# kubernetes-sigs/scheduler-plugins

Hardware: AMD Instinct MI355X
Metric: pod_x_node_filter_score_evals_per_sec (higher is better)
Workload: dtype f32+f64

## Files before the change

scheduler-plugins_amd/csrc/kernels_network.hip:

```cpp
#include <cstdlib>

#include "net_device.h"

namespace spx {

namespace {

using Acc = AccT<int>;


constexpr int kRowThreads = kNetRowThreads;
__global__ __launch_bounds__(kRowThreads) void k_net_cls(NetArgs g) {
  SPX_RESOLVE_ROWS(g);
  extern __shared__ __align__(16) int lds[];
  const int C = g.n_classes;
  int* cls_word = lds;
  int* cls_hosts = lds + C;
  uint32_t* cls_fin = reinterpret_cast<uint32_t*>(lds + 2 * C);
  unsigned* host_bits = reinterpret_cast<unsigned*>(lds + 3 * C);
  const int lane = threadIdx.x, nthr = blockDim.x;
  const int64_t pod = g.row_begin + blockIdx.x;
  if (pod >= g.row_end) return;
  const int key = g.pod_key[pod];
  const int flag = g.key_flag[key];
  const int lo = g.pair_ptr[key], hi = g.pair_end ? g.pair_end[key] : g.pair_ptr[key + 1];
  const int64_t n_words = (g.n_nodes + 31) / 32;
  const uint8_t* other0 = g.other_status[0] ? g.other_status[0] + pod * g.row_stride : nullptr;
  const uint8_t* other1 = g.other_status[1] ? g.other_status[1] + pod * g.row_stride : nullptr;
  uint8_t* out_st = g.out_status + pod * g.row_stride;
  uint8_t* out_sc = g.out_score + pod * g.row_stride;

  constexpr int kG = 16;
  const int64_t groups = g.row_stride / kG;
  uint16_t* scored = reinterpret_cast<uint16_t*>(host_bits + n_words);
  const bool fuse = g.out_alloc != nullptr && nthr == 64;
  uint8_t* out_al = fuse ? g.out_alloc + pod * g.row_stride : nullptr;
  auto load16 = [](const void* p) { return *reinterpret_cast<const uint4*>(p); };
  auto byte_of = [](const uint32_t (&w)[4], int j) { return (w[j >> 2] >> (8 * (j & 3))) & 0xffu; };
  auto half_of = [](const uint32_t (&w)[8], int j) { return (w[j >> 1] >> (16 * (j & 1))) & 0xffffu; };
  auto rel16 = [&](int64_t n0, uint32_t (&r)[16]) {
#pragma unroll
    for (int q = 0; q < 4; ++q) {
      const uint4 v = load16(g.alloc_rel + n0 + 4 * q);
      r[4 * q] = v.x, r[4 * q + 1] = v.y, r[4 * q + 2] = v.z, r[4 * q + 3] = v.w;
    }
  };
  auto others16 = [&](int64_t n0, uint32_t (&oth)[4]) {
    uint4 o4 = uint4{0, 0, 0, 0};
    if (other0) o4 = load16(other0 + n0);
    if (other1) {
      const uint4 v = load16(other1 + n0);
      o4.x |= v.x, o4.y |= v.y, o4.z |= v.z, o4.w |= v.w;
    }
    oth[0] = o4.x, oth[1] = o4.y, oth[2] = o4.z, oth[3] = o4.w;
  };
  auto open16 = [&](int64_t n0, const uint32_t (&oth)[4]) {
    uint32_t open = 0;
#pragma unroll
    for (int j = 0; j < kG; ++j) open |= (n0 + j < g.n_nodes && byte_of(oth, j) == 0u) ? 1u << j : 0u;
    return open;
  };
  auto wave_range = [&](uint32_t& lo32, uint32_t& hi32) {
    lo32 = static_cast<uint32_t>(wave_min(static_cast<int>(lo32 ^ 0x80000000u))) ^ 0x80000000u;
    hi32 = static_cast<uint32_t>(wave_max(static_cast<int>(hi32 ^ 0x80000000u))) ^ 0x80000000u;
  };
  auto alloc16 = [&](int64_t n0, uint32_t ok, uint32_t alo, double ab, uint32_t (&al_w)[4]) {
    uint32_t rel[16];
    rel16(n0, rel);
#pragma unroll
    for (int j = 0; j < kG; ++j)
      if ((ok >> j) & 1u) al_w[j >> 2] |= static_cast<uint32_t>(static_cast<double>(rel[j] - alo) * ab) << (8 * (j & 3));
  };

  if (flag != 0) {
    const uint32_t st = flag == 2 ? 0xffffffffu : 0u;
    uint32_t alo = 0xffffffffu, ahi = 0u;
    const bool fz = fuse && flag != 2;
    if (fz) {
      for (int64_t q = lane; q < groups; q += nthr) {
        const int64_t n0 = q * kG;
        uint32_t open = 0;
        if (n0 < g.n_nodes) {
          uint32_t oth[4], rel[16];
          others16(n0, oth);
          rel16(n0, rel);
          open = open16(n0, oth);
#pragma unroll
          for (int j = 0; j < kG; ++j)
            if ((open >> j) & 1u) alo = rel[j] < alo ? rel[j] : alo, ahi = rel[j] > ahi ? rel[j] : ahi;
        }
        scored[q] = static_cast<uint16_t>(open);
      }
      wave_range(alo, ahi);
    }
    const uint32_t arange = (fz && ahi >= alo) ? ahi - alo : 0u;
    const double ab = arange ? (100.0 / static_cast<double>(arange)) * (1.0 + 0x1p-49) : 0.0;
    for (int64_t q = lane; q < groups; q += nthr) {
      const int64_t n0 = q * kG;
      *reinterpret_cast<uint4*>(out_st + n0) = uint4{st, st, st, st};
      *reinterpret_cast<uint4*>(out_sc + n0) = uint4{0u, 0u, 0u, 0u};
      if (fuse) {
        uint32_t al_w[4] = {0, 0, 0, 0};
        const uint32_t ok = fz ? scored[q] : 0u;
        if (ok != 0 && arange != 0) alloc16(n0, ok, alo, ab, al_w);
        *reinterpret_cast<uint4*>(out_al + n0) = uint4{al_w[0], al_w[1], al_w[2], al_w[3]};
      }
    }
    return;
  }

  constexpr int kStage = kNetStagePairs;
  const int scored_words = static_cast<int>((g.row_stride / 16 + 1) / 2);
  long long* sp_max = reinterpret_cast<long long*>(lds + ((3 * C + static_cast<int>(n_words) + scored_words + 1) & ~1));
  int* sp_host = reinterpret_cast<int*>(sp_max + kStage);
  int* sp_region = sp_host + kStage;
  int* sp_zone = sp_region + kStage;
  const bool staged = nthr == kRowThreads && hi - lo <= kStage;
  const StagedPairs sp{sp_host, sp_region, sp_zone, sp_max, hi - lo};
  if (staged) {
    for (int i = lane; i < hi - lo; i += nthr) {
      const int host = g.pair_node[lo + i];
      sp_host[i] = host, sp_region[i] = g.region[host], sp_zone[i] = g.zone[host], sp_max[i] = g.pair_max[lo + i];
    }
    __syncthreads();
  }
  auto direct = [&](int64_t node) { return staged ? direct_eval_staged<int>(g, node, sp) : direct_eval<int>(g, node, lo, hi); };
  for (int c = lane; c < C; c += nthr) {
    Acc a{0, 0, 0};
    const int region = g.cls_region[c], zone = g.cls_zone[c];
    if (staged) {
      for (int i = 0; i < sp.n; ++i) add_pair(a, g, region, zone, sp_region[i], sp_zone[i], sp_max[i]);
    } else {
      for (int i = lo; i < hi; ++i) {
        const int host = g.pair_node[i];
        add_pair(a, g, region, zone, g.region[host], g.zone[host], g.pair_max[i]);
      }
    }
    cls_word[c] = a.cost | (a.vio > a.sat ? static_cast<int>(0x80000000u) : 0);
    cls_hosts[c] = 0;
  }
  for (int64_t w = lane; w < n_words; w += nthr) host_bits[w] = 0u;
  __syncthreads();
  for (int i = lo + lane; i < hi; i += nthr) {
    const int host = g.pair_node[i];
    const unsigned bit = 1u << (host & 31);
    if (!(atomicOr(&host_bits[host >> 5], bit) & bit)) atomicAdd(&cls_hosts[g.node_class16[host]], 1);
  }
  __syncthreads();

  auto classes16 = [&](int64_t n0, uint32_t (&cw)[8]) {
    const uint4 c0 = load16(g.node_class16 + n0), c1 = load16(g.node_class16 + n0 + 8);
    cw[0] = c0.x, cw[1] = c0.y, cw[2] = c0.z, cw[3] = c0.w, cw[4] = c1.x, cw[5] = c1.y, cw[6] = c1.z, cw[7] = c1.w;
  };
  auto hosts16 = [&](int64_t n0) -> uint32_t { return (host_bits[n0 >> 5] >> (n0 & 31)) & 0xffffu; };

  int mn = INT32_MAX, mx = INT32_MIN;
  uint32_t alo = 0xffffffffu, ahi = 0u;
  const bool walk = other0 || other1 || fuse;
  if (!walk) {
    for (int c = lane; c < C; c += nthr) {
      const int w = cls_word[c];
      if (w >= 0 && g.cls_size[c] - cls_hosts[c] > 0) {
        mn = w < mn ? w : mn;
        mx = w > mx ? w : mx;
      }
    }
    for (int i = lo + lane; i < hi; i += nthr) {
      const Acc a = direct(g.pair_node[i]);
      if (!(a.vio > a.sat)) {
        mn = a.cost < mn ? a.cost : mn;
        mx = a.cost > mx ? a.cost : mx;
      }
    }
  } else {
    for (int64_t q = lane; q < groups; q += nthr) {
      const int64_t n0 = q * kG;
      uint32_t ok = 0;
      if (n0 < g.n_nodes) {
        uint32_t oth[4], cw[8], rel[16];
        others16(n0, oth);
        classes16(n0, cw);
        if (fuse) rel16(n0, rel);
        const uint32_t hb = hosts16(n0);
        const uint32_t open = open16(n0, oth);
#pragma unroll
        for (int j = 0; j < kG; ++j) {
          const int w = cls_word[half_of(cw, j)];
          if (((open & ~hb) >> j) & 1u && w >= 0) {
            mn = w < mn ? w : mn;
            mx = w > mx ? w : mx;
            ok |= 1u << j;
            if (fuse) alo = rel[j] < alo ? rel[j] : alo, ahi = rel[j] > ahi ? rel[j] : ahi;
          }
        }
        for (uint32_t hs = open & hb; hs != 0; hs &= hs - 1) {
          const int j = __builtin_ctz(hs);
          const Acc a = direct(n0 + j);
          if (!(a.vio > a.sat)) {
            mn = a.cost < mn ? a.cost : mn;
            mx = a.cost > mx ? a.cost : mx;
            ok |= 1u << j;
            if (fuse) {
              const uint32_t r = g.alloc_rel[n0 + j];
              alo = r < alo ? r : alo, ahi = r > ahi ? r : ahi;
            }
          }
        }
      }
      scored[q] = static_cast<uint16_t>(ok);
    }
  }
  mn = wave_min(mn);
  mx = wave_max(mx);
  if (fuse) wave_range(alo, ahi);
  if (nthr > 64) {
    __shared__ int s_mn[kRowThreads / 64], s_mx[kRowThreads / 64];
    if ((lane & 63) == 0) s_mn[lane >> 6] = mn, s_mx[lane >> 6] = mx;
    __syncthreads();
    mn = INT32_MAX, mx = INT32_MIN;
    for (int w = 0; w < (nthr >> 6); ++w) {
      mn = s_mn[w] < mn ? s_mn[w] : mn;
      mx = s_mx[w] > mx ? s_mx[w] : mx;
    }
  }

  for (int c = lane; c < C; c += nthr) {
    const int w = cls_word[c];
    int score = w >= 0 ? norm_cost(w, mn, mx) : 0;
    score = score < 0 ? 0 : (score > 255 ? 255 : score);
    cls_fin[c] = static_cast<uint32_t>(score) | (w < 0 ? static_cast<uint32_t>(SPX_NET_ST_UNSCHEDULABLE) << 8 : 0u);
  }
  __syncthreads();
  const uint32_t arange = (fuse && ahi >= alo) ? ahi - alo : 0u;
  const double ab = arange ? (100.0 / static_cast<double>(arange)) * (1.0 + 0x1p-49) : 0.0;

  for (int64_t q = lane; q < groups; q += nthr) {
    const int64_t n0 = q * kG;
    uint32_t st_w[4] = {0, 0, 0, 0}, sc_w[4] = {0, 0, 0, 0}, al_w[4] = {0, 0, 0, 0};
    if (n0 < g.n_nodes) {
      const uint32_t ok = walk ? scored[q] : 0xffffu;
      uint32_t cw[8];
      classes16(n0, cw);
      const uint32_t hb = hosts16(n0);
#pragma unroll
      for (int j = 0; j < kG; ++j) {
        uint32_t fin = cls_fin[half_of(cw, j)];
        if (n0 + j >= g.n_nodes) fin = 0;
        st_w[j >> 2] |= (fin >> 8) << (8 * (j & 3));
        if ((ok >> j) & 1u) sc_w[j >> 2] |= (fin & 0xffu) << (8 * (j & 3));
      }
      for (uint32_t hs = hb; hs != 0; hs &= hs - 1) {
        const int j = __builtin_ctz(hs);
        if (n0 + j >= g.n_nodes) continue;
        const Acc a = direct(n0 + j);
        const bool pass = !(a.vio > a.sat);
        int score = pass ? norm_cost(a.cost, mn, mx) : 0;
        score = score < 0 ? 0 : (score > 255 ? 255 : score);
        const uint32_t sh = 8 * (j & 3), keep = ~(0xffu << sh);
        st_w[j >> 2] = (st_w[j >> 2] & keep) | ((pass ? 0u : static_cast<uint32_t>(SPX_NET_ST_UNSCHEDULABLE)) << sh);
        sc_w[j >> 2] = (sc_w[j >> 2] & keep) | ((((ok >> j) & 1u) ? static_cast<uint32_t>(score) : 0u) << sh);
      }
      if (fuse && ok != 0 && arange != 0) alloc16(n0, ok, alo, ab, al_w);
    }
    *reinterpret_cast<uint4*>(out_st + n0) = uint4{st_w[0], st_w[1], st_w[2], st_w[3]};
    *reinterpret_cast<uint4*>(out_sc + n0) = uint4{sc_w[0], sc_w[1], sc_w[2], sc_w[3]};
    if (fuse) *reinterpret_cast<uint4*>(out_al + n0) = uint4{al_w[0], al_w[1], al_w[2], al_w[3]};
  }
}

}

size_t net_lds_bytes(int n_classes, int64_t n_nodes) {
  return static_cast<size_t>(3 * n_classes) * sizeof(int) + static_cast<size_t>((n_nodes + 31) / 32) * sizeof(unsigned) +
         static_cast<size_t>((n_nodes + 4096) / 16 + 2) * sizeof(uint16_t) + 16;
}

bool launch_net(const NetArgs& g, hipStream_t s) {
  if (g.row_end <= g.row_begin) return false;
  if (g.cost_wide) {
    launch_net_wide(g, s);
    return false;
  }
  const unsigned blocks = static_cast<unsigned>(g.row_end - g.row_begin);
  size_t lds = g.n_classes > 0 ? net_lds_bytes(g.n_classes, g.n_nodes) : 16;
  if (blocks == 1) lds = ((lds + 7) & ~static_cast<size_t>(7)) + kNetStagePairs * (sizeof(long long) + 3 * sizeof(int));
  const bool generic_only = (g.opts & kOptNetGeneric) != 0;
  if (!generic_only && !g.out_raw && g.n_classes > 0 && g.n_classes <= 65535 && g.node_class16 && g.row_stride % 16 == 0) {
    NetArgs h = g;
    if (blocks == 1 || !h.alloc_rel) h.out_alloc = nullptr;
    hipLaunchKernelGGL(k_net_cls, dim3(blocks), dim3(blocks == 1 ? kRowThreads : 64), lds, s, h);
    return h.out_alloc != nullptr;
  }
  hipLaunchKernelGGL(k_net<int>, dim3(blocks), dim3(64), lds, s, g);
  return false;
}

}
```

Measured before the change: 4923 billion.

## Add templated multi-row class kernel with software-pipelined 16-node group loads

Adds a new per-row network kernel, templated on which other-status inputs exist and whether allocation scoring is fused, and launches it for multi-row batches. It processes 16-node groups with vector loads and double-buffers status, class and alloc-rel loads one burst ahead, computing min/max with branchless masks. The aim is to hide global load latency and remove runtime branches and per-byte work from the old generic path. In exchange it adds eight kernel instantiations, more register pressure, and a separate host-node fixup loop that must reproduce the old semantics exactly.

```diff
diff --git a/scheduler-plugins_amd/csrc/kernels_network.hip b/scheduler-plugins_amd/csrc/kernels_network.hip
--- a/scheduler-plugins_amd/csrc/kernels_network.hip
+++ b/scheduler-plugins_amd/csrc/kernels_network.hip
@@ -268,6 +268,343 @@
   }
 }
 
+constexpr int kGrp = 16;
+constexpr int kBurst = 4;
+constexpr int kBurstW = 1;
+
+__device__ __forceinline__ uint4 ld16(const void* p) { return *reinterpret_cast<const uint4*>(p); }
+__device__ __forceinline__ uint32_t word_of(const uint4& v, int i) { return i == 0 ? v.x : (i == 1 ? v.y : (i == 2 ? v.z : v.w)); }
+__device__ __forceinline__ uint32_t half16(const uint4& c0, const uint4& c1, int j) {
+  return (word_of(j < 8 ? c0 : c1, (j & 7) >> 1) >> (16 * (j & 1))) & 0xffffu;
+}
+__device__ __forceinline__ uint32_t mask_of_bit(uint32_t bits, int j) { return static_cast<uint32_t>(static_cast<int>(bits << (31 - j)) >> 31); }
+__device__ __forceinline__ uint32_t umin32(uint32_t a, uint32_t b) { return a < b ? a : b; }
+__device__ __forceinline__ uint32_t umax32(uint32_t a, uint32_t b) { return a > b ? a : b; }
+__device__ __forceinline__ uint32_t nonzero_bytes(uint32_t x) {
+  x |= x >> 4, x |= x >> 2, x |= x >> 1;
+  return ((x & 0x01010101u) * 0x01020408u) >> 24 & 0xfu;
+}
+__device__ __forceinline__ void pin(uint32_t& x) { asm volatile("" : "+v"(x)); }
+__device__ __forceinline__ void put_byte(uint4& v, int j, uint32_t b) {
+  const uint32_t s = b << (8 * (j & 3));
+  if ((j >> 2) == 0) v.x |= s;
+  else if ((j >> 2) == 1) v.y |= s;
+  else if ((j >> 2) == 2) v.z |= s;
+  else v.w |= s;
+}
+
+template <bool kO0, bool kO1, bool kFuse>
+__global__ __launch_bounds__(64) void k_net_cls_rows(NetArgs g) {
+  SPX_RESOLVE_ROWS(g);
+  extern __shared__ __align__(16) int lds[];
+  const int C = g.n_classes;
+  int* cls_word = lds;
+  int* cls_hosts = lds + C;
+  uint32_t* cls_fin = reinterpret_cast<uint32_t*>(lds + 2 * C);
+  unsigned* host_bits = reinterpret_cast<unsigned*>(lds + 3 * C);
+  const int lane = threadIdx.x;
+  const int64_t pod = g.row_begin + blockIdx.x;
+  if (pod >= g.row_end) return;
+  const int key = g.pod_key[pod];
+  const int flag = g.key_flag[key];
+  const int lo = g.pair_ptr[key], hi = g.pair_end ? g.pair_end[key] : g.pair_ptr[key + 1];
+  const int64_t n_words = (g.n_nodes + 31) / 32;
+  const uint8_t* other0 = kO0 ? g.other_status[0] + pod * g.row_stride : nullptr;
+  const uint8_t* other1 = kO1 ? g.other_status[1] + pod * g.row_stride : nullptr;
+  uint8_t* out_st = g.out_status + pod * g.row_stride;
+  uint8_t* out_sc = g.out_score + pod * g.row_stride;
+  uint8_t* out_al = kFuse ? g.out_alloc + pod * g.row_stride : nullptr;
+  const int groups = static_cast<int>(g.row_stride / kGrp);
+  const int qmax = static_cast<int>((g.n_nodes - 1) / kGrp);
+  const int n_nodes = static_cast<int>(g.n_nodes);
+  uint16_t* scored = reinterpret_cast<uint16_t*>(host_bits + n_words);
+  constexpr bool kWalk = kO0 || kO1 || kFuse;
+
+  auto group_of = [&](int b, int k, int per) { return (b * per + k) * 64 + lane; };
+  auto clamped = [&](int q) { return q < qmax ? q : qmax; };
+  auto inside_of = [&](int q) -> uint32_t {
+    const int left = q <= qmax ? n_nodes - q * kGrp : 0;
+    return left >= kGrp ? 0xffffu : (1u << left) - 1u;
+  };
+  auto bursts_of = [&](int per) { return (groups + 64 * per - 1) / (64 * per); };
+  auto issue_status = [&](int b, uint4 (&sa)[kBurst], uint4 (&sb)[kBurst]) {
+#pragma unroll
+    for (int k = 0; k < kBurst; ++k) {
+      const uint32_t off = static_cast<uint32_t>(clamped(group_of(b, k, kBurst))) * kGrp;
+      if constexpr (kO0) sa[k] = ld16(other0 + off);
+      if constexpr (kO1) sb[k] = ld16(other1 + off);
+    }
+  };
+  auto issue_classes = [&](int b, auto& c0, auto& c1) {
+    constexpr int per = sizeof(c0) / sizeof(c0[0]);
+#pragma unroll
+    for (int k = 0; k < per; ++k) {
+      const uint16_t* p = g.node_class16 + static_cast<uint32_t>(clamped(group_of(b, k, per))) * kGrp;
+      c0[k] = ld16(p), c1[k] = ld16(p + 8);
+    }
+  };
+  auto issue_rel = [&](int b, auto& r) {
+    constexpr int per = sizeof(r) / sizeof(r[0]);
+#pragma unroll
+    for (int k = 0; k < per; ++k) {
+      const uint32_t* p = static_cast<const uint32_t*>(__builtin_assume_aligned(g.alloc_rel + static_cast<uint32_t>(clamped(group_of(b, k, per))) * kGrp, 64));
+#pragma unroll
+      for (int i = 0; i < 4; ++i) r[k][i] = ld16(p + 4 * i);
+    }
+  };
+  auto open_of = [&](int q, const uint4& sa, const uint4& sb) -> uint32_t {
+    uint32_t open = inside_of(q);
+    if constexpr (kO0 || kO1) {
+      uint4 o = uint4{0, 0, 0, 0};
+      if constexpr (kO0) o = sa;
+      if constexpr (kO1) o.x |= sb.x, o.y |= sb.y, o.z |= sb.z, o.w |= sb.w;
+      open &= ~(nonzero_bytes(o.x) | nonzero_bytes(o.y) << 4 | nonzero_bytes(o.z) << 8 | nonzero_bytes(o.w) << 12);
+    }
+    return open;
+  };
+  auto wave_range = [&](uint32_t& lo32, uint32_t& hi32) {
+    lo32 = static_cast<uint32_t>(wave_min(static_cast<int>(lo32 ^ 0x80000000u))) ^ 0x80000000u;
+    hi32 = static_cast<uint32_t>(wave_max(static_cast<int>(hi32 ^ 0x80000000u))) ^ 0x80000000u;
+  };
+  auto alloc_cells = [&](const uint4 (&r)[4], uint32_t ok, uint32_t alo, double ab) {
+    uint4 al = uint4{0, 0, 0, 0};
+#pragma unroll
+    for (int j = 0; j < kGrp; ++j) {
+      const uint32_t d = (word_of(r[j >> 2], j & 3) - alo) & mask_of_bit(ok, j);
+      put_byte(al, j, static_cast<uint32_t>(static_cast<double>(d) * ab));
+      if ((j & 3) == 3) pin(al.x), pin(al.y), pin(al.z), pin(al.w);
+    }
+    return al;
+  };
+  uint32_t alo = 0xffffffffu, ahi = 0u;
+  uint4 s0a[kBurst] = {}, s0b[kBurst] = {}, s1a[kBurst] = {}, s1b[kBurst] = {};
+
+  if (flag != 0) {
+    const uint32_t st = flag == 2 ? 0xffffffffu : 0u;
+    const bool fz = kFuse && flag != 2;
+    if (fz) {
+      auto step = [&](int b, uint4 (&ca)[kBurst], uint4 (&cb)[kBurst], uint4 (&na)[kBurst], uint4 (&nb)[kBurst]) {
+        uint4 r[kBurst][4];
+        issue_rel(b, r);
+        issue_status(b + 1, na, nb);
+#pragma unroll
+        for (int k = 0; k < kBurst; ++k) {
+          const int q = group_of(b, k, kBurst);
+          const uint32_t open = open_of(q, ca[k], cb[k]);
+#pragma unroll
+          for (int j = 0; j < kGrp; ++j) {
+            const uint32_t v = word_of(r[k][j >> 2], j & 3), sel = mask_of_bit(open, j);
+            alo = umin32(alo, v | ~sel), ahi = umax32(ahi, v & sel);
+          }
+          if (q < groups) scored[q] = static_cast<uint16_t>(open);
+          pin(alo), pin(ahi);
+        }
+      };
+      const int nb = bursts_of(kBurst);
+      issue_status(0, s0a, s0b);
+      int b = 0;
+      for (; b + 1 < nb; b += 2) step(b, s0a, s0b, s1a, s1b), step(b + 1, s1a, s1b, s0a, s0b);
+      if (b < nb) step(b, s0a, s0b, s1a, s1b);
+      wave_range(alo, ahi);
+    }
+    const uint32_t arange = (fz && ahi >= alo) ? ahi - alo : 0u;
+    const double ab = arange ? (100.0 / static_cast<double>(arange)) * (1.0 + 0x1p-49) : 0.0;
+    const uint4 st4 = uint4{st, st, st, st}, zero4 = uint4{0u, 0u, 0u, 0u};
+    if (arange != 0) {
+      if constexpr (kFuse) {
+        auto step = [&](int b, uint4 (&cr)[kBurstW][4], uint4 (&nr)[kBurstW][4]) {
+          issue_rel(b + 1, nr);
+#pragma unroll
+          for (int k = 0; k < kBurstW; ++k) {
+            const int q = group_of(b, k, kBurstW);
+            const uint32_t ok = scored[clamped(q)] & inside_of(q);
+            const uint4 al = alloc_cells(cr[k], ok, alo, ab);
+            if (q < groups) {
+              *reinterpret_cast<uint4*>(out_st + static_cast<uint32_t>(q) * kGrp) = st4;
+              *reinterpret_cast<uint4*>(out_sc + static_cast<uint32_t>(q) * kGrp) = zero4;
+              *reinterpret_cast<uint4*>(out_al + static_cast<uint32_t>(q) * kGrp) = al;
+            }
+          }
+        };
+        uint4 r0[kBurstW][4], r1[kBurstW][4];
+        const int nb = bursts_of(kBurstW);
+        issue_rel(0, r0);
+        int b = 0;
+        for (; b + 1 < nb; b += 2) step(b, r0, r1), step(b + 1, r1, r0);
+        if (b < nb) step(b, r0, r1);
+      }
+    } else {
+      for (int q = lane; q < groups; q += 64) {
+        *reinterpret_cast<uint4*>(out_st + static_cast<uint32_t>(q) * kGrp) = st4;
+        *reinterpret_cast<uint4*>(out_sc + static_cast<uint32_t>(q) * kGrp) = zero4;
+        if constexpr (kFuse) *reinterpret_cast<uint4*>(out_al + static_cast<uint32_t>(q) * kGrp) = zero4;
+      }
+    }
+    return;
+  }
+
+  auto direct = [&](int64_t node) { return direct_eval<int>(g, node, lo, hi); };
+  for (int c = lane; c < C; c += 64) {
+    Acc a{0, 0, 0};
+    const int region = g.cls_region[c], zone = g.cls_zone[c];
+    for (int i = lo; i < hi; ++i) {
+      const int host = g.pair_node[i];
+      add_pair(a, g, region, zone, g.region[host], g.zone[host], g.pair_max[i]);
+    }
+    cls_word[c] = a.cost | (a.vio > a.sat ? static_cast<int>(0x80000000u) : 0);
+    cls_hosts[c] = 0;
+  }
+  for (int64_t w = lane; w < n_words; w += 64) host_bits[w] = 0u;
+  __syncthreads();
+  for (int i = lo + lane; i < hi; i += 64) {
+    const int host = g.pair_node[i];
+    const unsigned bit = 1u << (host & 31);
+    if (!(atomicOr(&host_bits[host >> 5], bit) & bit)) atomicAdd(&cls_hosts[g.node_class16[host]], 1);
+  }
+  __syncthreads();
+  auto hosts_of = [&](int qc) -> uint32_t { return (host_bits[qc >> 1] >> (16 * (qc & 1))) & 0xffffu; };
+
+  int mn = INT32_MAX, mx = INT32_MIN;
+  if constexpr (!kWalk) {
+    for (int c = lane; c < C; c += 64) {
+      const int w = cls_word[c];
+      if (w >= 0 && g.cls_size[c] - cls_hosts[c] > 0) {
+        mn = w < mn ? w : mn;
+        mx = w > mx ? w : mx;
+      }
+    }
+    for (int i = lo + lane; i < hi; i += 64) {
+      const Acc a = direct(g.pair_node[i]);
+      if (!(a.vio > a.sat)) {
+        mn = a.cost < mn ? a.cost : mn;
+        mx = a.cost > mx ? a.cost : mx;
+      }
+    }
+  } else {
+    uint32_t umn = INT32_MAX, umx = 0u, any = 0u;
+    auto step = [&](int b, uint4 (&ca)[kBurst], uint4 (&cb)[kBurst], uint4 (&na)[kBurst], uint4 (&nb)[kBurst]) {
+      uint4 c0[kBurst], c1[kBurst], r[kBurst][4];
+      issue_classes(b, c0, c1);
+      if constexpr (kFuse) issue_rel(b, r);
+      issue_status(b + 1, na, nb);
+#pragma unroll
+      for (int k = 0; k < kBurst; ++k) {
+        const int q = group_of(b, k, kBurst), qc = clamped(q);
+        const uint32_t open = open_of(q, ca[k], cb[k]);
+        const uint32_t hb = hosts_of(qc), cells = open & ~hb;
+        uint32_t ok = 0;
+#pragma unroll
+        for (int j = 0; j < kGrp; ++j) {
+          const uint32_t w = static_cast<uint32_t>(cls_word[half16(c0[k], c1[k], j)]);
+          const uint32_t sel = mask_of_bit(cells, j) & ~static_cast<uint32_t>(static_cast<int>(w) >> 31);
+          umn = umin32(umn, w | ~sel), umx = umax32(umx, w & sel);
+          ok = ok >> 1 | (sel & 0x8000u);
+          if constexpr (kFuse) {
+            const uint32_t v = word_of(r[k][j >> 2], j & 3);
+            alo = umin32(alo, v | ~sel), ahi = umax32(ahi, v & sel);
+          }
+        }
+        any |= ok;
+        pin(umn), pin(umx), pin(alo), pin(ahi);
+        if (q < groups) scored[q] = static_cast<uint16_t>(ok);
+      }
+    };
+    const int nb = bursts_of(kBurst);
+    issue_status(0, s0a, s0b);
+    int b = 0;
+    for (; b + 1 < nb; b += 2) step(b, s0a, s0b, s1a, s1b), step(b + 1, s1a, s1b, s0a, s0b);
+    if (b < nb) step(b, s0a, s0b, s1a, s1b);
+    if (any != 0) mn = static_cast<int>(umn), mx = static_cast<int>(umx);
+    for (int q = lane; q <= qmax; q += 64) {
+      uint32_t ok = scored[q];
+      for (uint32_t hs = hosts_of(q) & inside_of(q); hs != 0; hs &= hs - 1) {
+        const int j = __builtin_ctz(hs);
+        const int64_t node = static_cast<int64_t>(q) * kGrp + j;
+        bool open = true;
+        if constexpr (kO0) open = other0[node] == 0;
+        if constexpr (kO1) open = open && other1[node] == 0;
+        if (!open) continue;
+        const Acc a = direct(node);
+        if (!(a.vio > a.sat)) {
+          mn = a.cost < mn ? a.cost : mn;
+          mx = a.cost > mx ? a.cost : mx;
+          ok |= 1u << j;
+          if constexpr (kFuse) {
+            const uint32_t v = g.alloc_rel[node];
+            alo = v < alo ? v : alo, ahi = v > ahi ? v : ahi;
+          }
+        }
+      }
+      scored[q] = static_cast<uint16_t>(ok);
+    }
+  }
+  mn = wave_min(mn);
+  mx = wave_max(mx);
+  if constexpr (kFuse) wave_range(alo, ahi);
+
+  for (int c = lane; c < C; c += 64) {
+    const int w = cls_word[c];
+    int score = w >= 0 ? norm_cost(w, mn, mx) : 0;
+    score = score < 0 ? 0 : (score > 255 ? 255 : score);
+    cls_fin[c] = static_cast<uint32_t>(score) | (w < 0 ? static_cast<uint32_t>(SPX_NET_ST_UNSCHEDULABLE) << 8 : 0u);
+  }
+  __syncthreads();
+  const uint32_t arange = (kFuse && ahi >= alo) ? ahi - alo : 0u;
+  const double ab = arange ? (100.0 / static_cast<double>(arange)) * (1.0 + 0x1p-49) : 0.0;
+
+  auto step = [&](int b, uint4 (&cc0)[kBurstW], uint4 (&cc1)[kBurstW], uint4 (&cr)[kBurstW][4], uint4 (&nc0)[kBurstW], uint4 (&nc1)[kBurstW],
+                  uint4 (&nr)[kBurstW][4]) {
+    issue_classes(b + 1, nc0, nc1);
+    if constexpr (kFuse) issue_rel(b + 1, nr);
+#pragma unroll
+    for (int k = 0; k < kBurstW; ++k) {
+      const int q = group_of(b, k, kBurstW), qc = clamped(q);
+      const uint32_t inside = inside_of(q);
+      const uint32_t ok = (kWalk ? scored[qc] : 0xffffu) & inside;
+      uint4 st_w = uint4{0, 0, 0, 0}, sc_w = uint4{0, 0, 0, 0};
+#pragma unroll
+      for (int j = 0; j < kGrp; ++j) {
+        const uint32_t fin = cls_fin[half16(cc0[k], cc1[k], j)];
+        put_byte(st_w, j, fin >> 8 & mask_of_bit(inside, j));
+        put_byte(sc_w, j, fin & 0xffu & mask_of_bit(ok, j));
+      }
+      if (q < groups) {
+        *reinterpret_cast<uint4*>(out_st + static_cast<uint32_t>(q) * kGrp) = st_w;
+        *reinterpret_cast<uint4*>(out_sc + static_cast<uint32_t>(q) * kGrp) = sc_w;
+        if constexpr (kFuse) *reinterpret_cast<uint4*>(out_al + static_cast<uint32_t>(q) * kGrp) = alloc_cells(cr[k], ok, alo, ab);
+      }
+    }
+  };
+  uint4 c00[kBurstW], c01[kBurstW], c10[kBurstW], c11[kBurstW], r0[kBurstW][4], r1[kBurstW][4];
+  const int nb = bursts_of(kBurstW);
+  issue_classes(0, c00, c01);
+  if constexpr (kFuse) issue_rel(0, r0);
+  int b = 0;
+  for (; b + 1 < nb; b += 2) step(b, c00, c01, r0, c10, c11, r1), step(b + 1, c10, c11, r1, c00, c01, r0);
+  if (b < nb) step(b, c00, c01, r0, c10, c11, r1);
+  for (int q = lane; q <= qmax; q += 64) {
+    const uint32_t ok = kWalk ? scored[q] : 0xffffu;
+    for (uint32_t hs = hosts_of(q) & inside_of(q); hs != 0; hs &= hs - 1) {
+      const int j = __builtin_ctz(hs);
+      const int64_t node = static_cast<int64_t>(q) * kGrp + j;
+      const Acc a = direct(node);
+      const bool pass = !(a.vio > a.sat);
+      int score = pass ? norm_cost(a.cost, mn, mx) : 0;
+      score = score < 0 ? 0 : (score > 255 ? 255 : score);
+      out_st[node] = pass ? 0 : SPX_NET_ST_UNSCHEDULABLE;
+      out_sc[node] = ((ok >> j) & 1u) ? static_cast<uint8_t>(score) : 0;
+    }
+  }
+}
+
+using NetRowsKernel = void (*)(NetArgs);
+NetRowsKernel net_rows_kernel(bool o0, bool o1, bool fuse) {
+  static const NetRowsKernel k[8] = {k_net_cls_rows<false, false, false>, k_net_cls_rows<true, false, false>, k_net_cls_rows<false, true, false>,
+                                     k_net_cls_rows<true, true, false>,   k_net_cls_rows<false, false, true>, k_net_cls_rows<true, false, true>,
+                                     k_net_cls_rows<false, true, true>,   k_net_cls_rows<true, true, true>};
+  return k[(o0 ? 1 : 0) | (o1 ? 2 : 0) | (fuse ? 4 : 0)];
+}
+
 }
 
 size_t net_lds_bytes(int n_classes, int64_t n_nodes) {
@@ -288,7 +625,11 @@
   if (!generic_only && !g.out_raw && g.n_classes > 0 && g.n_classes <= 65535 && g.node_class16 && g.row_stride % 16 == 0) {
     NetArgs h = g;
     if (blocks == 1 || !h.alloc_rel) h.out_alloc = nullptr;
-    hipLaunchKernelGGL(k_net_cls, dim3(blocks), dim3(blocks == 1 ? kRowThreads : 64), lds, s, h);
+    if (blocks == 1 || g.n_nodes <= 0)
+      hipLaunchKernelGGL(k_net_cls, dim3(blocks), dim3(blocks == 1 ? kRowThreads : 64), lds, s, h);
+    else
+      hipLaunchKernelGGL(net_rows_kernel(h.other_status[0] != nullptr, h.other_status[1] != nullptr, h.out_alloc != nullptr), dim3(blocks), dim3(64),
+                         lds, s, h);
     return h.out_alloc != nullptr;
   }
   hipLaunchKernelGGL(k_net<int>, dim3(blocks), dim3(64), lds, s, g);
```

Result: no change. 4901 billion (-0.4%).
